# fgiral000/gencast-flax-nnx

Measured on AMD Instinct MI355X. Metric: denoiser-calls/sec, higher is better.
Workload: dtype f16x3 (every product = 3 fp16 MFMAs on hi/lo-split f32 operands: 22-bit products, f32 accumulate; f32 storage); 1 GPU; nano-GenCast DPM-Solver++2S 20-step sample, 2.5deg grid (73x144), 1 ensemble member per GPU, batch 1; dead_call_skipped=True, grid_nodes=10512, mesh_nodes=2562, latent=256, layers=16, heads=4, ffw_hidden=2048, c_in=262, c_out=82, k_hop=8, parallelism=ensemble-dp1, broadcast=none, rccl_ranks=0, precision=f16x3, library_built_from_this_tree=True, launcher=single

## Files before the change

### gencast-flax-nnx_amd/csrc/gc_api.hip

```cpp
#include <dlfcn.h>

#include "gc_handle.h"

using namespace gci;

namespace {

void protect_pending_noise(gc_handle* h) {
  if (h->guard_pending && h->d_noise == h->last_noise) std::swap(h->d_noise, h->d_noise_alt);
}

int check_ready(gc_handle* h) {
  if (!h) return GC_ERR_INVALID_ARGUMENT;
  if (!h->finalized) return fail(h, GC_ERR_STATE, "gc_finalize has not been called");
  return GC_OK;
}

struct Rccl {
  void* lib = nullptr;
  ncclResult_t (*GetUniqueId)(ncclUniqueId*) = nullptr;
  ncclResult_t (*CommInitRank)(ncclComm_t*, int, ncclUniqueId, int) = nullptr;
  ncclResult_t (*CommDestroy)(ncclComm_t) = nullptr;
  ncclResult_t (*CommCount)(const ncclComm_t, int*) = nullptr;
  ncclResult_t (*CommUserRank)(const ncclComm_t, int*) = nullptr;
// ... 104 lines not shown
  return hipDeviceGetPCIBusId(out, (int)cap, device_id) == hipSuccess ? GC_OK : GC_ERR_HIP;
}

const char* gc_last_error(const gc_handle* h) { return h ? h->err.c_str() : g_create_error.c_str(); }

static void read_switches(gc_handle* h) {
  auto is = [](const char* name, const char* value) { const char* v = std::getenv(name); return v && std::string(v) == value; };
  auto off = [](const char* name) { const char* v = std::getenv(name); return v && *v && std::atoi(v) == 0; };
  auto on = [](const char* name) { const char* v = std::getenv(name); return v && *v == '1'; };
  h->f16x3 = !is("GC_PRECISION", "f32");
  h->use_graphs = !is("GC_TUNE_GRAPH", "0");
  h->m2g_fuse_sum = !off("GC_TUNE_M2G_FUSE_SUM");
  h->embed_cache = !off("GC_TUNE_EMBED_CACHE");
  h->attn_items = !off("GC_TUNE_ATTN_ITEMS");
  h->mlp_pair = !off("GC_TUNE_MLP_PAIR");
  h->edge_terms = !off("GC_TUNE_EDGE_TERMS");
  h->a16 = !off("GC_TUNE_A16");
  h->graph_serialize = on("GC_TUNE_GRAPH_SERIALIZE");
  h->graph_verbose = on("GC_TUNE_GRAPH_VERBOSE");
  h->poison = on("GC_DEBUG_POISON");
}

int gc_create(const gc_config* cfg, int device_id, gc_handle** out) {
  return guarded(nullptr, [&]() -> int {
  if (!cfg || !out) { g_create_error = "null argument"; return GC_ERR_INVALID_ARGUMENT; }
  *out = nullptr;
  const gc_config& c = *cfg;
  auto bad = [&](const char* m) { g_create_error = m; return GC_ERR_INVALID_ARGUMENT; };
  if (c.latent_size <= 0 || c.d_model <= 0 || c.num_heads <= 0 || c.ffw_hidden <= 0 ||
      c.num_layers < 0 || c.c_in <= 0 || c.c_out <= 0 || c.batch <= 0)
    return bad("all dimensions must be positive");
// ... 1228 lines not shown
```

### gencast-flax-nnx_amd/csrc/gc_forward.hip

```cpp
#include "gc_handle.h"

namespace gci {

template <class To, class From>
static const To& a16_view(const From& v) {
  static_assert(sizeof(To) == sizeof(From), "argument struct mismatch between the two kernel builds");
  return reinterpret_cast<const To&>(v);
}

Route make_route(const gc_handle* h) {
  const int D = h->cfg.d_model, F = h->cfg.ffw_hidden;
  Route r;
  r.f16 = h->f16x3 && !h->weights_f16_unsafe && !h->in_fallback;
  r.x32 = !r.f16 && h->f32_ws;
  const bool streams = r.f16 || r.x32;
  r.ffw_slabs = streams ? h->ffw_fused_slabs : 0;
  r.st16 = h->feat16 && h->a16 && r.f16 && D % 128 == 0 && D <= 512 &&
           (h->ffw_fused_slabs > 0 || (F % 128 == 0 && (F / h->ffw2_splits) % 128 == 0));
  r.v2 = r.f16 && r.ws(3 * D, D, 1);
  r.att_items = (h->att_n_items > 0 && r.ws(3 * D, D, 1) && h->attn_splits == 1 && D <= 512) ? h->att_n_items : 0;
  r.fuse_row = streams && D % 128 == 0 && D <= 512;
  r.node_ws = r.f16;
  r.split_edge = h->split_edge;
  r.try_pair = h->mlp_pair && h->hidden_layers == 1;
  r.m2g_fused = h->m2g_fuse_sum && h->hg.m2g_tri && h->hidden_layers == 1 && streams;
  r.embed_cache = h->embed_cache_live && h->embed_cache_ready && !h->feat16 && h->hidden_layers == 1 && streams;
  r.edge_terms = h->embed_cache_live && h->terms.ready && edge_terms_possible(h) && r.f16;
  return r;
}

bool edge_terms_possible(const gc_handle* h) {
  return h->edge_terms && h->f16x3 && !h->weights_f16_unsafe && !h->in_fallback && !h->feat16 && h->hidden_layers == 1 &&
         h->cfg.latent_size == 256 && h->cfg.batch == 1 && h->hg.m2g_tri;
}

static gc::Segment seg(const float* ptr, const int* index, const float* affine, int width, int ld, int bcast) {
  gc::Segment s;
  s.ptr = ptr; s.index = index; s.affine = affine; s.width = width; s.ld = ld; s.bcast = bcast;
  return s;
}

struct MlpCall {
// ... 13 lines not shown
                        const float* residual = nullptr) {
  MlpCall c;
  c.rows = rows; c.B = B; c.out = out; c.ldo = ldo; c.residual = residual;
  return c.segments(segs);
}

static int build_mlp_args(gc_handle* h, const DevMlp& w, const MlpCall& c, gc::MlpArgs* out_args) {
  const Route& r = h->route;
  gc::MlpArgs& a = *out_args;
  a = gc::MlpArgs{};
  a.nseg = c.nseg; a.nadd = c.nadd;
  std::copy(c.seg, c.seg + c.nseg, a.seg);
  std::copy(c.add, c.add + c.nadd, a.add);
  a.rows = c.rows; a.B = c.B; a.hidden = h->cfg.latent_size;
  a.f16 = r.f16 ? 1 : 0;
  const Weight& w1 = c.nadd ? w.w1e : w.w1;
  a.w1t = pick(w1, r, Form::Staged); a.ldw1 = w1.ld; a.b1 = w.b1;
  a.w2t = pick(w.w2, r, Form::Staged); a.b2 = w.b2;
  if (r.f16 || r.x32) {
    a.w1f = pick(w1, r, Form::Streaming); a.k1f = w1.kf;
    a.w2f = pick(w.w2, r, Form::Streaming); a.ones = h->d_ones; a.zeros = h->d_zeros;
    a.f32w = r.x32 ? 1 : 0;
  }
  a.n_out = w.n_out; a.n_out_pad = w.n_out_pad; a.do_ln = c.ln ? 1 : 0;
  a.cond = (c.cond && w.cond_off >= 0) ? (h->cond_cur ? h->cond_cur : h->d_cond) + w.cond_off : nullptr;
  a.cond_stride = h->cond_total;
  a.residual = c.residual; a.out = c.out; a.ldo = c.ldo;
  a.round16 = h->feat16 ? 1 : 0;
  a.round_out = (h->feat16 && c.round_out) ? 1 : 0;
  a.a16 = r.st16 ? 1 : 0;
  a.seg0_f32 = c.seg0_f32 ? 1 : 0;
  a.out_f32 = c.out_f32 ? 1 : 0;
  a.tri = c.tri ? 1 : 0;
  if (c.tri && !gc::mlp_runs_weight_streaming(a))
    return fail(h, GC_ERR_INTERNAL, "the triple-sum epilogue exists in the weight-streaming MLP kernel only");
  return GC_OK;
}

static int enqueue_mlp(gc_handle* h, const gc::MlpArgs& a) {
  return launch(h, gc::KC_MLP, [&] {
    return a.a16 ? gc_a16::launch_mlp(h->stream, a16_view<gc_a16::MlpArgs>(a)) : gc::launch_mlp(h->stream, a);
  });
}
static int enqueue_mlp_pair(gc_handle* h, const gc::MlpArgs& a, const gc::MlpArgs& b) {
  return launch(h, gc::KC_MLP, [&] {
    return a.a16 ? gc_a16::launch_mlp_pair(h->stream, a16_view<gc_a16::MlpArgs>(a), a16_view<gc_a16::MlpArgs>(b))
                 : gc::launch_mlp_pair(h->stream, a, b);
  });
}
static int enqueue_gemm_ws(gc_handle* h, int cls, const gc::GemmArgs& ga, int mt, int splits, int epi) {
  return launch(h, cls, [&] {
    return ga.a16 ? gc_a16::launch_gemm_ws(h->stream, cls, a16_view<gc_a16::GemmArgs>(ga), mt, splits, epi)
                  : gc::launch_gemm_ws(h->stream, cls, ga, mt, splits, epi);
  });
}
static int enqueue_gemm_rowop(gc_handle* h, int cls, const gc::GemmArgs& ga, const gc::RowFuse& rf) {
  return launch(h, cls, [&] {
    return ga.a16 ? gc_a16::launch_gemm_rowop(h->stream, cls, a16_view<gc_a16::GemmArgs>(ga), a16_view<gc_a16::RowFuse>(rf))
                  : gc::launch_gemm_rowop(h->stream, cls, ga, rf);
  });
}
static int enqueue_ffw_fused(gc_handle* h, const gc::FfwArgs& fa) {
// ... 86 lines not shown
static int node_gemm(gc_handle* h, const float* nodes, int rows, const Weight& w, float* out) {
  const Route& r = h->route;
  const int L = h->cfg.latent_size;
  gc::GemmArgs ga{};
  ga.a = nodes; ga.lda = L; ga.a_f32 = 1; ga.ldw = L;
  ga.rows = rows; ga.n = L; ga.k_slice = L; ga.bias = nullptr; ga.act = 0; ga.out = out; ga.ldo = L;
  ga.round16 = 0;
  ga.out_f32 = 1;
  if (r.node_ws) {
    ga.wt = pick(w, r, Form::Streaming); ga.a16 = r.st16 ? 1 : 0;
    return enqueue_gemm_ws(h, gc::KC_GEMM_NODE, ga, pick_ws_mt(rows, L, 1), 1, 0);
  }
  ga.wt = pick(w, r, Form::Staged);
  return launch(h, gc::KC_GEMM_NODE, [&] { return gc::launch_gemm(h->stream, gc::KC_GEMM_NODE, ga, 1, 0, r.f16); });
}
static int edge_node_products(gc_handle* h, const DevMlp& w, const float* senders, int snd_rows, float* snd_out,
                              const float* receivers, int rcv_rows, float* rcv_out) {
  if (int rc = node_gemm(h, senders, snd_rows, w.w1snd, snd_out)) return rc;
  return node_gemm(h, receivers, rcv_rows, w.w1rcv, rcv_out);
}

static MlpCall edge_call(gc_handle* h, const float* e_hat, const float* e_affine, int E, const int* snd, const int* rcv,
                         const float* nsnd, const float* nrcv, const float* psnd, const float* prcv, float* out) {
  const int B = h->cfg.batch, L = h->cfg.latent_size;
  MlpCall c = mlp_call({seg(e_hat, nullptr, e_affine, L, L, 1)}, E * B, B, out, L);
  c.seg0_f32 = true;
  if (h->route.split_edge) c.add_terms({{psnd, snd}, {prcv, rcv}});
  else c.segments({seg(nsnd, snd, nullptr, L, L, 0), seg(nrcv, rcv, nullptr, L, L, 0)});
  return c;
}
// ... 65 lines not shown
                                  : mlp_call({seg(h->d_xp, nullptr, nullptr, h->kp, h->kp, 0)}, g.G * B, B, h->d_g0, L);
    embed.seg0_f32 = true;
    if (r.embed_cache) embed.add_terms({{h->d_pstat, nullptr}});
    if ((rc = run_mlp(h, r.embed_cache ? h->g2m_embed_grid_n : h->g2m_embed_grid, embed))) return rc;
  }
  const size_t ML = (size_t)g.M * L;
  if (r.edge_terms && (h->term_slot < 0 || !h->terms.ready))
    return fail(h, GC_ERR_INTERNAL, "edge terms: the forward has no slot of the cache");
  const float* const m0 = r.edge_terms ? h->terms.m0 + h->term_slot * ML : h->d_m0;
  h->m0_cur = m0;
  if (!r.edge_terms && (rc = launch(h, gc::KC_PACK, [&] {
         return gc::launch_affine_rows(s, h->d_m0_hat, cond + h->g2m_embed_mesh.cond_off, cs, g.M, B, L,
                                       h->d_m0, h->feat16, r.st16);
       })))
    return rc;
  if (r.edge_terms && (rc = node_gemm(h, h->d_g0, g.G * B, h->g2m_edge.w1snd, h->d_pg))) return rc;
  const MlpCall edge = r.edge_terms
                           ? edge_terms_call(h, h->terms.T1 + (size_t)h->term_slot * g.E1 * L, g.E1, h->d_g2m_snd, h->d_g2m_rcv,
                                             h->d_pg, h->terms.Pm + h->term_slot * ML, h->d_e1)
                           : edge_call(h, h->d_e0_hat, cond + h->g2m_embed_edge.cond_off, g.E1, h->d_g2m_snd, h->d_g2m_rcv,
                                       h->d_g0, h->d_m0, h->d_pg, h->d_pm, h->d_e1);
  const MlpCall node = mlp_call({seg(h->d_g0, nullptr, nullptr, L, L, 0)}, g.G * B, B, h->d_g1, L, h->d_g0);
  gc::MlpArgs ea{}, na{};
  bool paired = false;
  if (r.try_pair) {
    if ((rc = build_mlp_args(h, h->g2m_edge, edge, &ea)) || (rc = build_mlp_args(h, h->g2m_grid, node, &na))) return rc;
    paired = gc::mlp_pair_supported(ea, na);
  }
  if (r.split_edge && (rc = edge_node_products(h, h->g2m_edge, h->d_g0, g.G * B, h->d_pg, h->d_m0, g.M * B, h->d_pm)))
    return rc;
  if ((rc = paired ? enqueue_mlp_pair(h, ea, na) : run_mlp(h, h->g2m_edge, edge))) return rc;
  if ((rc = launch(h, gc::KC_SEGSUM, [&] {
         return gc::launch_segsum(s, h->d_e1, h->d_g2m_ptr, h->d_g2m_eid, g.M, g.E1, B, L, h->d_agg1, h->feat16, r.st16,
                                  h->g2m_agg_norm);
       })))
    return rc;
  if ((rc = run_mlp(h, h->g2m_mesh, mlp_call({seg(m0, nullptr, nullptr, L, L, 0), seg(h->d_agg1, nullptr, nullptr, L, L, 0)},
// ... 151 lines not shown
  const gc::HostGraph& g = h->hg;
  const gc_config& c = h->cfg;
  const size_t L = c.latent_size, n = distinct.size();
  const size_t per_slot = ((size_t)g.E1 + g.E2 + 2 * (size_t)g.M) * L;
  t.bytes = (int64_t)(n * per_slot * sizeof(float));
  if (n == 0 || n > (size_t)gc::kMaxSigmaList || t.bytes > h->edge_term_cap_mb * (int64_t)(1 << 20) ||
      n * (size_t)c.batch * h->cond_total > h->cond_all_cap) {
    t.bytes = 0;
    return GC_OK;
  }
  int rc;
  BufferGroup* own = &h->term_allocs;
  if ((rc = dev_alloc(h, &t.T1, n * g.E1 * L, own)) || (rc = dev_alloc(h, &t.T2, n * g.E2 * L, own)) ||
      (rc = dev_alloc(h, &t.m0, n * g.M * L, own)) || (rc = dev_alloc(h, &t.Pm, n * g.M * L, own)))
    return rc;
  hipStream_t s = h->stream;
  h->route = make_route(h);
  gc::SigmaList sl{};
  for (size_t i = 0; i < n; ++i) sl.v[i] = distinct[i];
  if ((rc = launch(h, gc::KC_COND, [&] {
         return gc::launch_cond_multi(s, sl, (int)n, c.batch, h->d_nw0t, h->d_nb0, h->d_nw1t, h->d_nb1, c.noise_num_frequencies,
                                      c.noise_hidden, c.noise_base_period, h->d_wc_all, h->d_bc_all, h->cond_total, h->d_cond_all);
       })))
    return rc;
  const int cs = h->cond_total;
  for (size_t i = 0; i < n; ++i) {
    const float* cond = h->d_cond_all + i * (size_t)c.batch * cs;
    const struct { const float* hat; int cond_off, items; float* staged; const Weight* w; float* out; } passes[] = {
        {h->d_e0_hat, h->g2m_embed_edge.cond_off, g.E1, h->d_e1, &h->g2m_edge.w1e, t.T1 + i * g.E1 * L},
        {h->d_f0_hat, h->m2g_embed_edge.cond_off, g.E2, h->d_f1, &h->m2g_edge.w1e, t.T2 + i * g.E2 * L},
// ... 15 lines not shown
```

### gencast-flax-nnx_amd/csrc/gc_handle.h

```cpp
#pragma once
#include <hip/hip_runtime.h>

#include <algorithm>
#include <array>
#include <cmath>
#include <cstdio>
#include <cstdlib>
#include <cstring>
#include <map>
#include <memory>
#include <mutex>
#include <string>
#include <type_traits>
#include <vector>

#include <rccl/rccl.h>

#include "../../include/gencast_hip.h"
#include "../../include/gencast_hip_debug.h"
#include "gc_graph.h"
#include "gc_kernels.h"

namespace gci {

// ... 1 lines not shown

struct Route {
  bool f16 = false;
  bool x32 = false;
  bool st16 = false;
  int ffw_slabs = 0;
  bool v2 = false;
  int att_items = 0;
  bool fuse_row = false;
  bool node_ws = false;
  bool m2g_fused = false;
  bool split_edge = false;
  bool try_pair = false;
  bool embed_cache = false;
  bool edge_terms = false;
  bool ws(int n, int k, int splits) const { return (f16 || x32) && n % 128 == 0 && (k / splits) % 128 == 0; }
};

struct Weight {
  float* t = nullptr;
  float* s = nullptr;
  float* f = nullptr;
  float* x = nullptr;
  int ld = 0, kf = 0;
};
enum class Form { Staged, Streaming };
inline const float* pick(const Weight& w, const Route& r, Form form) {
  if (form == Form::Streaming) return r.x32 ? w.x : w.f;
  return r.f16 ? w.s : w.t;
}
// ... 115 lines not shown
  float *d_wc_all = nullptr, *d_bc_all = nullptr;

  float *d_m0_hat = nullptr, *d_e0_hat = nullptr, *d_f0_hat = nullptr;

  int kp = 0;
  float *d_sigma = nullptr, *d_condvec = nullptr, *d_cond = nullptr;
  float* d_cond_all = nullptr;
  size_t cond_all_cap = 0;
  const float* cond_cur = nullptr;
  float *d_feats = nullptr, *d_xp = nullptr, *d_g0 = nullptr, *d_g1 = nullptr, *d_m0 = nullptr,
        *d_x = nullptr, *d_e1 = nullptr, *d_agg1 = nullptr, *d_qkv = nullptr, *d_att = nullptr,
        *d_u = nullptr, *d_m2 = nullptr, *d_f1 = nullptr, *d_agg2 = nullptr, *d_g2 = nullptr,
        *d_y = nullptr, *d_h = nullptr, *d_part = nullptr, *d_apart_o = nullptr, *d_apart_ml = nullptr,
        *d_pg = nullptr, *d_pm = nullptr;
  bool mlp_pair = true;
  bool embed_cache = true;
  bool embed_cache_ready = false;
  bool embed_cache_live = false;
  int nwp = 0;
  float *d_xn = nullptr, *d_pstat = nullptr;
  float *w1st_t = nullptr, *w1st_s = nullptr;
  gci::DevMlp g2m_embed_grid_n;
  std::vector<int> h_slots;
  int64_t embed_cache_samples = 0;
  bool m2g_fuse_sum = true;
  struct EdgeTerms {
    bool ready = false;
    std::vector<float> sigmas;
    std::vector<int> call_slot;
    float *T1 = nullptr, *T2 = nullptr, *m0 = nullptr, *Pm = nullptr;
    int64_t bytes = 0;
  };
  bool edge_terms = true;
  int64_t edge_term_cap_mb = 4096;
  EdgeTerms terms;
  gci::BufferGroup term_allocs{groups};
  int term_slot = -1;
  const float* m0_cur = nullptr;
  int64_t edge_term_samples = 0;
  float *d_ones = nullptr, *d_zeros = nullptr;
  int hidden_layers = 1;
  float* d_mlp_tmp[2] = {nullptr, nullptr};
  float *d_feats2 = nullptr, *d_ro_a = nullptr, *d_ro_b = nullptr, *d_ro_forc = nullptr;
  int *d_ro_kind = nullptr, *d_ro_src = nullptr, *d_ro_sidx = nullptr;
  int ro_nforc = -1, ro_forc_cap = 0;
  bool has_sample = false;
  int max_tile_chunks = 0;
  int ffw_fused_slabs = 0;
// ... 463 lines not shown
```

### gencast-flax-nnx_amd/csrc/gc_kernels.hip

```cpp
#include "gc_kernels.h"

#include <algorithm>
#include <atomic>
#include <type_traits>

#include <math.h>
#include <stdlib.h>

#ifdef GC_TU_A16
#define GC_TU_NS gc_a16
#else
#define GC_TU_NS gc
#endif
namespace GC_TU_NS {
#ifdef GC_TU_A16
constexpr bool kTuA16 = true;
#else
constexpr bool kTuA16 = false;
#endif

#include "gc_dev_common.inc"


struct DynLdsOnce {
// ... 1034 lines not shown
          if (c + e < n) a.out[(size_t)orow * a.ldo + c + e] = v[e];
      }
    }
  }
  });
}

template <int NT1, int NT2, int MT, int WM, int NWC = 4, int NW2 = NWC,
          int OCC = mlp_ws_occ<NT1, WM, NWC>() , bool A16 = false,
          bool F32 = false, bool TERMS = false>
__global__ __launch_bounds__(64 * NWC * WM, OCC) void gc_mlp_ws_kernel(MlpArgs a) {
  gc_mlp_ws_body<NT1, NT2, MT, WM, NWC, NW2, OCC, A16, F32, TERMS>(a, (int)blockIdx.x);
}

template <int NT1, int NT2, int MT, int WM, int NWC = 4, int NW2 = NWC,
          int OCC = mlp_ws_occ<NT1, WM, NWC>(), bool A16 = false, bool F32 = false, bool TERMS_A = false >
__global__ __launch_bounds__(64 * NWC * WM, OCC) void gc_mlp_ws_pair_kernel(MlpArgs a, MlpArgs b, int na) {
  if ((int)blockIdx.x < na) gc_mlp_ws_body<NT1, NT2, MT, WM, NWC, NW2, OCC, A16, F32, TERMS_A>(a, (int)blockIdx.x);
  else gc_mlp_ws_body<NT1, NT2, MT, WM, NWC, NW2, OCC, A16, F32>(b, (int)blockIdx.x - na);
}

template <int NT1, int NT2, int MT, int WM, int NWC, int NW2>
static hipError_t mlp_ws_geometry(const MlpArgs& a, int* grid_out, size_t* lds_out) {
  constexpr int HID = NT1 * 32 * NWC, NPAD = NT2 * 32 * NW2, BM = 32 * MT * WM;
  constexpr int abuf = 2 * BM * ((BM >= 128 ? 64 : 128) + 4);
  constexpr int region = (abuf > BM * (HID + 4)) ? abuf : BM * (HID + 4);
  static_assert(BM * (NPAD + 4) <= region, "output tile must fit the shared region");
  *lds_out = (size_t)(6 * BM + region) * sizeof(float);
  if (a.nadd < 0 || a.nadd > 3 || (a.nadd > 0 && !a.add[0].ptr) || (a.nadd > 1 && !a.add[1].ptr) || (a.nadd > 2 && !a.add[2].ptr))
    return hipErrorInvalidValue;
  if (a.nseg != 0 && a.nadd > 2) return hipErrorInvalidValue;
  int ksum = 0;
  for (int i = 0; i < a.nseg; ++i) {
    if (a.seg[i].width % 32 || a.seg[i].ld % 4) return hipErrorInvalidValue;
// ... 11 lines not shown
      if (h16 && (a.seg[i].affine || a.seg[i].ld % 8 || a.seg[i].width % 8)) return hipErrorInvalidValue;
      if (a.nseg > 1 && a.seg[i].width % KCc) return hipErrorInvalidValue;
    }
  }
  int grid = (a.rows + BM - 1) / BM;
  if (a.tri) {
    if (a.rows % 3 || a.residual || a.ldo % 4 || a.n_out % 4 ||
        (a.cond && ((reinterpret_cast<size_t>(a.cond) & 15) || a.cond_stride % 4)))
      return hipErrorInvalidValue;
    grid = (a.rows / 3 + BM / 3 - 1) / (BM / 3);
  }
  *grid_out = grid;
  return hipSuccess;
}

template <int NT1, int NT2, int MT, int WM, int NWC = 4, int NW2 = NWC, bool TERMS_A = false>
static hipError_t launch_mlp_ws_pair_t(hipStream_t s, const MlpArgs& a, const MlpArgs& b) {
  int ga = 0, gb = 0;
  size_t lds = 0;
  if (hipError_t e = mlp_ws_geometry<NT1, NT2, MT, WM, NWC, NW2>(a, &ga, &lds)) return e;
  if (hipError_t e = mlp_ws_geometry<NT1, NT2, MT, WM, NWC, NW2>(b, &gb, &lds)) return e;
  constexpr int OCC = mlp_ws_occ<NT1, WM, NWC>();
  if ((a.nseg == 0) != TERMS_A || b.nseg == 0) return hipErrorInvalidValue;
  if constexpr (TERMS_A) {
    if constexpr (kTuA16) return hipErrorInvalidValue;
    else {
      static DynLdsOnce once_t;
      if (hipError_t e = once_t.ensure((const void*)gc_mlp_ws_pair_kernel<NT1, NT2, MT, WM, NWC, NW2, OCC, false, false, true>, (int)lds)) return e;
      hipLaunchKernelGGL((gc_mlp_ws_pair_kernel<NT1, NT2, MT, WM, NWC, NW2, OCC, false, false, true>), dim3(ga + gb),
                         dim3(64 * NWC * WM), lds, s, a, b, ga);
      return hipGetLastError();
    }
  }
  if constexpr (!kTuA16) {
    if (a.f32w) {
      static DynLdsOnce once32;
      if (hipError_t e = once32.ensure((const void*)gc_mlp_ws_pair_kernel<NT1, NT2, MT, WM, NWC, NW2, OCC, false, true>, (int)lds)) return e;
      hipLaunchKernelGGL((gc_mlp_ws_pair_kernel<NT1, NT2, MT, WM, NWC, NW2, OCC, false, true>), dim3(ga + gb),
                         dim3(64 * NWC * WM), lds, s, a, b, ga);
      return hipGetLastError();
    }
  }
  static DynLdsOnce once;
  if (hipError_t e = once.ensure((const void*)gc_mlp_ws_pair_kernel<NT1, NT2, MT, WM, NWC, NW2, OCC, kTuA16>, (int)lds)) return e;
  hipLaunchKernelGGL((gc_mlp_ws_pair_kernel<NT1, NT2, MT, WM, NWC, NW2, OCC, kTuA16>), dim3(ga + gb),
                     dim3(64 * NWC * WM), lds, s, a, b, ga);
  return hipGetLastError();
}

template <int NT1, int NT2, int MT, int WM, int NWC = 4, int NW2 = NWC, bool TERMS = false>
static hipError_t launch_mlp_ws_t(hipStream_t s, const MlpArgs& a) {
  int grid = 0;
  size_t lds = 0;
  if (hipError_t e = mlp_ws_geometry<NT1, NT2, MT, WM, NWC, NW2>(a, &grid, &lds)) return e;
  constexpr int OCC = mlp_ws_occ<NT1, WM, NWC>();
  if ((a.nseg == 0) != TERMS) return hipErrorInvalidValue;
  if constexpr (TERMS) {
    if constexpr (kTuA16) return hipErrorInvalidValue;
    else {
      static DynLdsOnce once_t;
      if (hipError_t e = once_t.ensure((const void*)gc_mlp_ws_kernel<NT1, NT2, MT, WM, NWC, NW2, OCC, false, false, true>, (int)lds)) return e;
// ... 58 lines not shown
  if (a.f16 || a.a16 || a.tri || !a.w1t || a.nadd < 0 || a.nadd > 2 || a.nseg == 0) return hipErrorInvalidValue;
  for (int i = 0; i < a.nadd; ++i)
    if (!a.add[i].index) return hipErrorInvalidValue;
#define GC_MLP(A_, B_) \
  if (nt1 == A_ && nt2 == B_) return launch_mlp_t<A_, B_, false, 1>(s, a);
  GC_MLP(1, 1) GC_MLP(2, 2) GC_MLP(2, 1) GC_MLP(4, 4) GC_MLP(4, 1)
#undef GC_MLP
  return hipErrorInvalidValue;
}

bool mlp_pair_supported(const MlpArgs& a, const MlpArgs& b) {
  auto ok = [](const MlpArgs& m) {
    if (!mlp_runs_weight_streaming(m) || m.tri || m.n_out_pad != m.hidden) return false;
    return m.hidden == 512 || (m.hidden == 256 && m.rows < kMlpMt2Rows);
  };
  if (b.nseg == 0 || (a.nseg == 0 && a.hidden != 256)) return false;
  return ok(a) && ok(b) && a.hidden == b.hidden && a.f16 == b.f16 && a.f32w == b.f32w && a.a16 == b.a16;
}
hipError_t launch_mlp_pair(hipStream_t s, const MlpArgs& a, const MlpArgs& b) {
  if (!mlp_pair_supported(a, b)) return hipErrorInvalidValue;
  if (a.hidden == 512) return launch_mlp_ws_pair_t<2, 2, 2, 1, 8, 8>(s, a, b);
  if (a.nseg == 0) return launch_mlp_ws_pair_t<1, 1, 1, 1, 8, 8, true>(s, a, b);
  return launch_mlp_ws_pair_t<1, 1, 1, 1, 8, 8>(s, a, b);
}

template <bool H16>
__device__ __forceinline__ f32x4 seg_ld4(const float* base, size_t elem) {
  if constexpr (H16) return ldh4(as_h16(base) + elem);
  else return ld4(base + elem);
}
template <bool H16>
__device__ __forceinline__ void seg_st4(float* base, size_t elem, f32x4 v) {
  if constexpr (H16) sth4(as_h16(base) + elem, v);
  else st4(base + elem, v);
}

template <bool H16>
__global__ __launch_bounds__(256) void gc_segsum_kernel(const float* __restrict__ src,
// ... 753 lines not shown
        }
        if (grow < g.rows) {
          if (g.out_f32) st4(g.out + (size_t)grow * g.ldo + cb + 8 * j, v);
          else sth4(as_h16(g.out) + (size_t)grow * g.ldo + cb + 8 * j, v);
        }
      }
    }
#ifdef GC_STAMPS
    stamp_out();
#endif
    return;
  }
  float bias_v = bias_reg;
  asm volatile("" : "+v"(bias_v));
  float* obase = (EPI == 1 ? g.out + (size_t)z * g.rows * g.ldo : g.out) + ntile * BN + wave * 32 + r;
  auto emit = [&](auto full_c, auto act_c, auto rnd_c) {
    constexpr bool FULL = decltype(full_c)::value, ACT = decltype(act_c)::value, RND = decltype(rnd_c)::value;
#pragma unroll
    for (int mt = 0; mt < MT; ++mt) {
      const int row0 = mtile * BM + mt * 32;
#pragma unroll
      for (int q = 0; q < 16; ++q) {
        float v = hilo(acc[mt][q], acc2[mt][q]);
        const int grow = row0 + acc_row(q, hh);
        if (EPI != 1) {
          v += bias_v;
          if (ACT) v = gelu_tanh_fast(v);
        }
        if (!F32 && CLS == KC_GEMM_QKV && EPI == 0) v = (fabsf(v) <= kF16Max) ? v : __builtin_nanf("");
        if (EPI != 1) v = r16_c<RND>(v);
// ... 12 lines not shown
  else emit(std::false_type{}, std::false_type{}, std::false_type{});
#ifdef GC_STAMPS
  stamp_out();
#endif
}

template <int CLS>
static hipError_t launch_gemm_ws_c(hipStream_t s, const GemmArgs& g_in, int mt, int splits, int epi) {
  if ((mt != 1 && mt != 2) || epi < 0 || (epi > 1 && epi != 3)) return hipErrorInvalidValue;
  if (epi == 3 && (CLS != KC_GEMM_QKV || !g_in.kv16 || g_in.kv_d % 32 || g_in.n != 3 * g_in.kv_d || splits != 1 ||
                   g_in.att_S > 0 || g_in.bias))
    return hipErrorInvalidValue;
  const int KC = mt == 1 ? 256 : 128;
  const int kc = g_in.k_slice < KC ? g_in.k_slice : KC;
  if (g_in.n % 128 || kc % 64 || g_in.k_slice % 128 || g_in.k_slice % kc || g_in.lda % 4 || g_in.ldw % 16 || splits < 1)
    return hipErrorInvalidValue;
  GemmArgs g = g_in;
  g.splits = splits;
  const int BM = 32 * mt;
  const int total = ((g.rows + BM - 1) / BM) * (g.n / 128) * splits;
  if (total <= 0) return hipSuccess;
  dim3 grid((total + 7) / 8 * 8), block(256);
#define GC_WS(MT_, EPI_, AM_) \
  hipLaunchKernelGGL((gc_gemm_ws_kernel<MT_, EPI_, CLS, AM_, 4, 3, kTuA16, (kTuA16 && AM_ == 0 && MT_ == 2)>), grid, block, 0, s, g);
  if constexpr (!kTuA16) {
    if (g.f32w) {
#define GC_WS32(MT_, EPI_, AM_) hipLaunchKernelGGL((gc_gemm_ws_kernel<MT_, EPI_, CLS, AM_, 4, 3, false, false, true>), grid, block, 0, s, g);
      if (epi == 3) return hipErrorInvalidValue;
      if (g.att_S > 0) {
        if (mt != 1 || epi != 1 || g.att_S > kMaxAttnSplits) return hipErrorInvalidValue;
// ... 1726 lines not shown
```

### gencast-flax-nnx_amd/csrc/gc_kernels_decl.inc

```
namespace GC_KERNELS_NS {

enum KernelClass : int {
  KC_COND = 0,
  KC_PACK,
  KC_MLP,
  KC_SEGSUM,
  KC_ROWOP,
  KC_GEMM_QKV,
  KC_ATTN,
  KC_ATTN_COMBINE,
  KC_GEMM_OUT,
  KC_GEMM_FFW1,
  KC_GEMM_FFW2,
  KC_GEMM_NODE,
  KC_NOISE,
  KC_COUNT
};

constexpr int kTileM = 32;
constexpr int kCondDim = 16;

struct Segment {
  const float* ptr;
  const int* index;
// ... 48 lines not shown
hipError_t launch_cond(hipStream_t s, const float* sigma_dev, float sigma_scalar, int B,
                       const float* w0t, const float* b0, const float* w1t, const float* b1,
                       int nfreq, int nhid, float base_period,
                       const float* wc_all, const float* bc_all, int total, float* cond_vec,
                       float* cond_out);

constexpr int kMaxSigmaList = 96;
struct SigmaList { float v[kMaxSigmaList]; };
hipError_t launch_cond_multi(hipStream_t s, const SigmaList& sl, int ncalls, int B, const float* w0t,
                             const float* b0, const float* w1t, const float* b1, int nfreq, int nhid,
                             float base_period, const float* wc_all, const float* bc_all, int total,
                             float* cond_out);

hipError_t launch_mlp(hipStream_t s, const MlpArgs& a);
bool mlp_pair_supported(const MlpArgs& a, const MlpArgs& b);
hipError_t launch_mlp_pair(hipStream_t s, const MlpArgs& a, const MlpArgs& b);

hipError_t launch_segsum(hipStream_t s, const float* src, const int* rowptr, const int* eids,
                         int n_items, int n_edges, int B, int width, float* out, bool round16 = false,
                         bool h16 = false ,
                         float norm = 0.f );

struct GemmArgs {
  const float* a;
  int lda;
  int a_f32;
  const float* att_po;
  const float* att_pml;
  int att_S, att_B, att_H, att_DH;
  const int* att_tiles;
  const float* wt;
  int ldw;
  int rows, n;
  int k_slice;
  int splits;
  const float* bias;
  int act;
  float* out;
  int ldo;
  int round16;
  int a16;
  void* kv16;
  int kv_d;
  int out_f32;
  int f32w;
};
hipError_t launch_gemm(hipStream_t s, int cls, const GemmArgs& g, int splits, int epi, bool f16);
hipError_t launch_gemm_ws(hipStream_t s, int cls, const GemmArgs& g, int mt, int splits, int epi);
#ifdef GC_STAMPS
hipError_t set_gemm_ws_stamp_buffer(unsigned long long* p);
#endif

struct FfwArgs {
  const float* a;
  int rows, d, f;
  const float* w1f;
  const float* b1;
  const float* w2f;
  float* out;
  int round16;
// ... 92 lines not shown
```

### gencast-flax-nnx_amd/csrc/gc_weights.hip

```cpp
#include "gc_handle.h"

namespace gci {

const char* const P_NOISE = "denoiser.noise_level_encoder";
const char* const P_G2M = "denoiser.predictor.grid2mesh_gnn";
const char* const P_M2G = "denoiser.predictor.mesh2grid_gnn";
const char* const P_TR = "denoiser.predictor.mesh_gnn.batch_first_transformer";

void add_mlp_specs(gc_handle* h, const std::string& p, int n_in, int n_hid, int n_out, bool cond) {
  const int nh = h->hidden_layers;
  for (int i = 0; i < nh; ++i) {
    const std::string l = p + ".network.network.layers." + std::to_string(2 * i);
    h->specs[l + ".kernel"] = {i == 0 ? n_in : n_hid, n_hid};
    h->specs[l + ".bias"] = {n_hid};
  }
  const std::string l = p + ".network.network.layers." + std::to_string(2 * nh);
  h->specs[l + ".kernel"] = {n_hid, n_out};
  h->specs[l + ".bias"] = {n_out};
  if (cond) {
    h->specs[p + ".norm_conditioning_layer.conditional_linear_layer.kernel"] = {gc::kCondDim, 2 * n_out};
    h->specs[p + ".norm_conditioning_layer.conditional_linear_layer.bias"] = {2 * n_out};
  }
}

// ... 241 lines not shown
  if ((rc = dev_upload(h, &n.w1e.f, encode_wf16(wn, L, k1e), own))) return rc;
  if (h->f32_ws && (rc = dev_upload(h, &n.w1e.x, encode_wf32(wn, L, k1e), own))) return rc;
  if (!h->d_xn) {
    const size_t GB = (size_t)h->hg.G * c.batch;
    if ((rc = dev_alloc(h, &h->d_xn, GB * h->nwp))) return rc;
    if ((rc = dev_alloc(h, &h->d_pstat, GB * L))) return rc;
    GC_HIP(h, hipMemset(h->d_xn, 0, GB * h->nwp * sizeof(float)));
  }
  h->embed_cache_ready = true;
  return GC_OK;
}

void free_weights(gc_handle* h) {
  (void)drop_edge_terms(h);
  h->weight_allocs.free();
  h->finalized = h->finalized_weights = h->embed_cache_ready = false;
  h->cond_cur = nullptr;
}

int finalize_weights(gc_handle* h) {
  const gc_config& c = h->cfg;
  const int L = c.latent_size, D = c.d_model, F = c.ffw_hidden;
  const std::string g = P_G2M, m = P_M2G, t = P_TR, nz = P_NOISE;
  BufferGroup* own = &h->weight_allocs;
  CondPacker cp;
  int rc;
  const int node_in = 3 + c.c_in;
  const std::string gn = g + ".processor_networks.0.graph_network";
  const std::string gn2 = m + ".processor_networks.0.graph_network";
  if (h->hidden_layers >= 2) {
// ... 10 lines not shown
  if ((rc = upload_mlp(h, gn + ".update_edge_fns.grid2mesh.edge_fn", 3 * L, 0, 3 * L, 3 * L, L, L, true, &cp, &h->g2m_edge))) return rc;
  if ((rc = upload_mlp(h, gn + ".update_node_fns.mesh_nodes.node_fn", 2 * L, 0, 2 * L, 2 * L, L, L, true, &cp, &h->g2m_mesh))) return rc;
  if ((rc = upload_mlp(h, gn + ".update_node_fns.grid_nodes.node_fn", L, 0, L, L, L, L, true, &cp, &h->g2m_grid))) return rc;
  if ((rc = upload_mlp(h, m + ".embedder_network.embed_edge_fns.mesh2grid", 4, 0, 4, 32, L, L, true, &cp, &h->m2g_embed_edge))) return rc;
  if ((rc = upload_mlp(h, gn2 + ".update_edge_fns.mesh2grid.edge_fn", 3 * L, 0, 3 * L, 3 * L, L, L, true, &cp, &h->m2g_edge))) return rc;
  if ((rc = upload_mlp(h, gn2 + ".update_node_fns.grid_nodes.node_fn", 2 * L, 0, 2 * L, 2 * L, L, L, true, &cp, &h->m2g_grid))) return rc;
  if ((rc = upload_mlp(h, m + ".decoder_network.embed_node_fns.grid_nodes", L, 0, L, L, L, c.c_out, false, &cp, &h->m2g_dec))) return rc;

  for (DevMlp* em : {&h->g2m_edge, &h->m2g_edge}) {
    const std::string pth = (em == &h->g2m_edge) ? gn + ".update_edge_fns.grid2mesh.edge_fn"
                                                 : gn2 + ".update_edge_fns.mesh2grid.edge_fn";
    const auto& k1 = h->weights.at(pth + ".network.network.layers.0.kernel");
    if ((rc = upload_weight(h, transpose_pad(k1, 3 * L, L, 0, L, L, L), L, L, L, h->f32_ws, &em->w1e))) return rc;
    if ((rc = upload_weight(h, transpose_pad(k1, 3 * L, L, L, L, L, L), L, L, L, false, &em->w1snd))) return rc;
    if ((rc = upload_weight(h, transpose_pad(k1, 3 * L, L, 2 * L, L, L, L), L, L, L, false, &em->w1rcv))) return rc;
  }
  h->layers.assign(c.num_layers, DevLayer());
  for (int i = 0; i < c.num_layers; ++i) {
    const std::string b = t + ".blocks." + std::to_string(i);
    DevLayer& ly = h->layers[i];
    auto wt = [&](const char* name, int n_in, int n_out) {
      return transpose_pad(h->weights.at(b + name), n_in, n_out, 0, n_in, n_in, n_out);
    };
    std::vector<float> qkv((size_t)3 * D * D);
    int part = 0;
    for (const char* q : {"q", "k", "v"}) {
      const auto tt = wt((std::string(".attn_module.") + q + "_proj.linear.kernel").c_str(), D, D);
      std::copy(tt.begin(), tt.end(), qkv.begin() + (size_t)part++ * D * D);
    }
    if ((rc = upload_weight(h, qkv, 3 * D, D, D, h->f32_ws, &ly.wqkv))) return rc;
// ... 46 lines not shown
```

Before: 781.2 calls/s.

## Fuse grid-node first-layer GEMM with edge sender products and reorder MLP pair blocks

Concatenates the grid2mesh edge sender weight and the grid node MLP first-layer weight into one image. One node GEMM with a split output now produces both the sender products and a precomputed node term Pn. The grid node MLP then consumes Pn as an add-term rather than recomputing its first layer, and the pair kernel gains a form where both halves use terms. It also adds an option to launch the heavier (terms-form or larger-K) half of an MLP pair first, to improve block scheduling. The change adds a buffer of size G×L and more template instantiations, and it changes the block-index mapping in the pair kernel.

```diff
diff --git a/gencast-flax-nnx_amd/csrc/gc_api.hip b/gencast-flax-nnx_amd/csrc/gc_api.hip
--- a/gencast-flax-nnx_amd/csrc/gc_api.hip
+++ b/gencast-flax-nnx_amd/csrc/gc_api.hip
@@ -142,7 +142,9 @@
   h->embed_cache = !off("GC_TUNE_EMBED_CACHE");
   h->attn_items = !off("GC_TUNE_ATTN_ITEMS");
   h->mlp_pair = !off("GC_TUNE_MLP_PAIR");
+  h->pair_order = !off("GC_TUNE_PAIR_ORDER");
   h->edge_terms = !off("GC_TUNE_EDGE_TERMS");
+  h->node_terms = !off("GC_TUNE_NODE_TERMS");
   h->a16 = !off("GC_TUNE_A16");
   h->graph_serialize = on("GC_TUNE_GRAPH_SERIALIZE");
   h->graph_verbose = on("GC_TUNE_GRAPH_VERBOSE");
diff --git a/gencast-flax-nnx_amd/csrc/gc_forward.hip b/gencast-flax-nnx_amd/csrc/gc_forward.hip
--- a/gencast-flax-nnx_amd/csrc/gc_forward.hip
+++ b/gencast-flax-nnx_amd/csrc/gc_forward.hip
@@ -26,6 +26,7 @@
   r.m2g_fused = h->m2g_fuse_sum && h->hg.m2g_tri && h->hidden_layers == 1 && streams;
   r.embed_cache = h->embed_cache_live && h->embed_cache_ready && !h->feat16 && h->hidden_layers == 1 && streams;
   r.edge_terms = h->embed_cache_live && h->terms.ready && edge_terms_possible(h) && r.f16;
+  r.node_terms = r.edge_terms && h->node_terms && h->w1sn_f && h->terms.Pn;
   return r;
 }
 
@@ -69,7 +70,7 @@
   std::copy(c.add, c.add + c.nadd, a.add);
   a.rows = c.rows; a.B = c.B; a.hidden = h->cfg.latent_size;
   a.f16 = r.f16 ? 1 : 0;
-  const Weight& w1 = c.nadd ? w.w1e : w.w1;
+  const Weight& w1 = (c.nadd && w.w1e.kf) ? w.w1e : w.w1;
   a.w1t = pick(w1, r, Form::Staged); a.ldw1 = w1.ld; a.b1 = w.b1;
   a.w2t = pick(w.w2, r, Form::Staged); a.b2 = w.b2;
   if (r.f16 || r.x32) {
@@ -98,9 +99,10 @@
   });
 }
 static int enqueue_mlp_pair(gc_handle* h, const gc::MlpArgs& a, const gc::MlpArgs& b) {
+  const bool b_first = h->pair_order && gc::mlp_pair_second_leads(a, b);
   return launch(h, gc::KC_MLP, [&] {
-    return a.a16 ? gc_a16::launch_mlp_pair(h->stream, a16_view<gc_a16::MlpArgs>(a), a16_view<gc_a16::MlpArgs>(b))
-                 : gc::launch_mlp_pair(h->stream, a, b);
+    return a.a16 ? gc_a16::launch_mlp_pair(h->stream, a16_view<gc_a16::MlpArgs>(a), a16_view<gc_a16::MlpArgs>(b), b_first)
+                 : gc::launch_mlp_pair(h->stream, a, b, b_first);
   });
 }
 static int enqueue_gemm_ws(gc_handle* h, int cls, const gc::GemmArgs& ga, int mt, int splits, int epi) {
@@ -217,6 +219,15 @@
   ga.wt = pick(w, r, Form::Staged);
   return launch(h, gc::KC_GEMM_NODE, [&] { return gc::launch_gemm(h->stream, gc::KC_GEMM_NODE, ga, 1, 0, r.f16); });
 }
+static int node_gemm2(gc_handle* h, const float* nodes, int rows, const float* image, float* out_a, float* out_b) {
+  const int L = h->cfg.latent_size;
+  gc::GemmArgs ga{};
+  ga.a = nodes; ga.lda = L; ga.a_f32 = 1; ga.ldw = L;
+  ga.rows = rows; ga.n = 2 * L; ga.k_slice = L; ga.bias = nullptr; ga.act = 0; ga.out = out_a; ga.ldo = L;
+  ga.out2 = out_b; ga.n_out1 = L;
+  ga.round16 = 0; ga.out_f32 = 1; ga.wt = image;
+  return enqueue_gemm_ws(h, gc::KC_GEMM_NODE, ga, pick_ws_mt(rows, 2 * L, 1), 1, 0);
+}
 static int edge_node_products(gc_handle* h, const DevMlp& w, const float* senders, int snd_rows, float* snd_out,
                               const float* receivers, int rcv_rows, float* rcv_out) {
   if (int rc = node_gemm(h, senders, snd_rows, w.w1snd, snd_out)) return rc;
@@ -312,13 +323,19 @@
                                        h->d_m0, h->feat16, r.st16);
        })))
     return rc;
-  if (r.edge_terms && (rc = node_gemm(h, h->d_g0, g.G * B, h->g2m_edge.w1snd, h->d_pg))) return rc;
+  if (r.edge_terms && (rc = r.node_terms ? node_gemm2(h, h->d_g0, g.G * B, h->w1sn_f, h->d_pg, h->terms.Pn)
+                                         : node_gemm(h, h->d_g0, g.G * B, h->g2m_edge.w1snd, h->d_pg)))
+    return rc;
   const MlpCall edge = r.edge_terms
                            ? edge_terms_call(h, h->terms.T1 + (size_t)h->term_slot * g.E1 * L, g.E1, h->d_g2m_snd, h->d_g2m_rcv,
                                              h->d_pg, h->terms.Pm + h->term_slot * ML, h->d_e1)
                            : edge_call(h, h->d_e0_hat, cond + h->g2m_embed_edge.cond_off, g.E1, h->d_g2m_snd, h->d_g2m_rcv,
                                        h->d_g0, h->d_m0, h->d_pg, h->d_pm, h->d_e1);
-  const MlpCall node = mlp_call({seg(h->d_g0, nullptr, nullptr, L, L, 0)}, g.G * B, B, h->d_g1, L, h->d_g0);
+  MlpCall node = mlp_call({seg(h->d_g0, nullptr, nullptr, L, L, 0)}, g.G * B, B, h->d_g1, L, h->d_g0);
+  if (r.node_terms) {
+    node = mlp_call({}, g.G * B, B, h->d_g1, L, h->d_g0);
+    node.add_terms({{h->terms.Pn, nullptr}});
+  }
   gc::MlpArgs ea{}, na{};
   bool paired = false;
   if (r.try_pair) {
@@ -500,6 +517,7 @@
   if ((rc = dev_alloc(h, &t.T1, n * g.E1 * L, own)) || (rc = dev_alloc(h, &t.T2, n * g.E2 * L, own)) ||
       (rc = dev_alloc(h, &t.m0, n * g.M * L, own)) || (rc = dev_alloc(h, &t.Pm, n * g.M * L, own)))
     return rc;
+  if (h->node_terms && h->w1sn_f && (rc = dev_alloc(h, &t.Pn, (size_t)g.G * c.batch * L, own))) return rc;
   hipStream_t s = h->stream;
   h->route = make_route(h);
   gc::SigmaList sl{};
diff --git a/gencast-flax-nnx_amd/csrc/gc_handle.h b/gencast-flax-nnx_amd/csrc/gc_handle.h
--- a/gencast-flax-nnx_amd/csrc/gc_handle.h
+++ b/gencast-flax-nnx_amd/csrc/gc_handle.h
@@ -39,6 +39,7 @@
   bool try_pair = false;
   bool embed_cache = false;
   bool edge_terms = false;
+  bool node_terms = false;
   bool ws(int n, int k, int splits) const { return (f16 || x32) && n % 128 == 0 && (k / splits) % 128 == 0; }
 };
 
@@ -184,6 +185,7 @@
         *d_y = nullptr, *d_h = nullptr, *d_part = nullptr, *d_apart_o = nullptr, *d_apart_ml = nullptr,
         *d_pg = nullptr, *d_pm = nullptr;
   bool mlp_pair = true;
+  bool pair_order = true;
   bool embed_cache = true;
   bool embed_cache_ready = false;
   bool embed_cache_live = false;
@@ -199,9 +201,12 @@
     std::vector<float> sigmas;
     std::vector<int> call_slot;
     float *T1 = nullptr, *T2 = nullptr, *m0 = nullptr, *Pm = nullptr;
+    float* Pn = nullptr;
     int64_t bytes = 0;
   };
   bool edge_terms = true;
+  bool node_terms = true;
+  float* w1sn_f = nullptr;
   int64_t edge_term_cap_mb = 4096;
   EdgeTerms terms;
   gci::BufferGroup term_allocs{groups};
diff --git a/gencast-flax-nnx_amd/csrc/gc_kernels.hip b/gencast-flax-nnx_amd/csrc/gc_kernels.hip
--- a/gencast-flax-nnx_amd/csrc/gc_kernels.hip
+++ b/gencast-flax-nnx_amd/csrc/gc_kernels.hip
@@ -1072,10 +1072,12 @@
 }
 
 template <int NT1, int NT2, int MT, int WM, int NWC = 4, int NW2 = NWC,
-          int OCC = mlp_ws_occ<NT1, WM, NWC>(), bool A16 = false, bool F32 = false, bool TERMS_A = false >
-__global__ __launch_bounds__(64 * NWC * WM, OCC) void gc_mlp_ws_pair_kernel(MlpArgs a, MlpArgs b, int na) {
-  if ((int)blockIdx.x < na) gc_mlp_ws_body<NT1, NT2, MT, WM, NWC, NW2, OCC, A16, F32, TERMS_A>(a, (int)blockIdx.x);
-  else gc_mlp_ws_body<NT1, NT2, MT, WM, NWC, NW2, OCC, A16, F32>(b, (int)blockIdx.x - na);
+          int OCC = mlp_ws_occ<NT1, WM, NWC>(), bool A16 = false, bool F32 = false, bool TERMS_A = false ,
+          bool TERMS_B = false >
+__global__ __launch_bounds__(64 * NWC * WM, OCC) void gc_mlp_ws_pair_kernel(MlpArgs a, MlpArgs b, int na, int a0, int b0) {
+  const int ta = (int)blockIdx.x - a0;
+  if ((unsigned)ta < (unsigned)na) gc_mlp_ws_body<NT1, NT2, MT, WM, NWC, NW2, OCC, A16, F32, TERMS_A>(a, ta);
+  else gc_mlp_ws_body<NT1, NT2, MT, WM, NWC, NW2, OCC, A16, F32, TERMS_B>(b, (int)blockIdx.x - b0);
 }
 
 template <int NT1, int NT2, int MT, int WM, int NWC, int NW2>
@@ -1117,21 +1119,23 @@
   return hipSuccess;
 }
 
-template <int NT1, int NT2, int MT, int WM, int NWC = 4, int NW2 = NWC, bool TERMS_A = false>
-static hipError_t launch_mlp_ws_pair_t(hipStream_t s, const MlpArgs& a, const MlpArgs& b) {
+template <int NT1, int NT2, int MT, int WM, int NWC = 4, int NW2 = NWC, bool TERMS_A = false, bool TERMS_B = false>
+static hipError_t launch_mlp_ws_pair_t(hipStream_t s, const MlpArgs& a, const MlpArgs& b, bool b_first) {
   int ga = 0, gb = 0;
   size_t lds = 0;
   if (hipError_t e = mlp_ws_geometry<NT1, NT2, MT, WM, NWC, NW2>(a, &ga, &lds)) return e;
   if (hipError_t e = mlp_ws_geometry<NT1, NT2, MT, WM, NWC, NW2>(b, &gb, &lds)) return e;
   constexpr int OCC = mlp_ws_occ<NT1, WM, NWC>();
-  if ((a.nseg == 0) != TERMS_A || b.nseg == 0) return hipErrorInvalidValue;
+  static_assert(TERMS_A || !TERMS_B, "a second half in the terms form: only beside a first one");
+  if ((a.nseg == 0) != TERMS_A || (b.nseg == 0) != TERMS_B) return hipErrorInvalidValue;
+  const int a0 = b_first ? gb : 0, b0 = b_first ? 0 : ga;
   if constexpr (TERMS_A) {
     if constexpr (kTuA16) return hipErrorInvalidValue;
     else {
       static DynLdsOnce once_t;
-      if (hipError_t e = once_t.ensure((const void*)gc_mlp_ws_pair_kernel<NT1, NT2, MT, WM, NWC, NW2, OCC, false, false, true>, (int)lds)) return e;
-      hipLaunchKernelGGL((gc_mlp_ws_pair_kernel<NT1, NT2, MT, WM, NWC, NW2, OCC, false, false, true>), dim3(ga + gb),
-                         dim3(64 * NWC * WM), lds, s, a, b, ga);
+      if (hipError_t e = once_t.ensure((const void*)gc_mlp_ws_pair_kernel<NT1, NT2, MT, WM, NWC, NW2, OCC, false, false, true, TERMS_B>, (int)lds)) return e;
+      hipLaunchKernelGGL((gc_mlp_ws_pair_kernel<NT1, NT2, MT, WM, NWC, NW2, OCC, false, false, true, TERMS_B>), dim3(ga + gb),
+                         dim3(64 * NWC * WM), lds, s, a, b, ga, a0, b0);
       return hipGetLastError();
     }
   }
@@ -1140,14 +1144,14 @@
       static DynLdsOnce once32;
       if (hipError_t e = once32.ensure((const void*)gc_mlp_ws_pair_kernel<NT1, NT2, MT, WM, NWC, NW2, OCC, false, true>, (int)lds)) return e;
       hipLaunchKernelGGL((gc_mlp_ws_pair_kernel<NT1, NT2, MT, WM, NWC, NW2, OCC, false, true>), dim3(ga + gb),
-                         dim3(64 * NWC * WM), lds, s, a, b, ga);
+                         dim3(64 * NWC * WM), lds, s, a, b, ga, a0, b0);
       return hipGetLastError();
     }
   }
   static DynLdsOnce once;
   if (hipError_t e = once.ensure((const void*)gc_mlp_ws_pair_kernel<NT1, NT2, MT, WM, NWC, NW2, OCC, kTuA16>, (int)lds)) return e;
   hipLaunchKernelGGL((gc_mlp_ws_pair_kernel<NT1, NT2, MT, WM, NWC, NW2, OCC, kTuA16>), dim3(ga + gb),
-                     dim3(64 * NWC * WM), lds, s, a, b, ga);
+                     dim3(64 * NWC * WM), lds, s, a, b, ga, a0, b0);
   return hipGetLastError();
 }
 
@@ -1236,14 +1240,19 @@
     if (!mlp_runs_weight_streaming(m) || m.tri || m.n_out_pad != m.hidden) return false;
     return m.hidden == 512 || (m.hidden == 256 && m.rows < kMlpMt2Rows);
   };
-  if (b.nseg == 0 || (a.nseg == 0 && a.hidden != 256)) return false;
+  if ((a.nseg == 0 && a.hidden != 256) || (b.nseg == 0 && a.nseg != 0)) return false;
   return ok(a) && ok(b) && a.hidden == b.hidden && a.f16 == b.f16 && a.f32w == b.f32w && a.a16 == b.a16;
 }
-hipError_t launch_mlp_pair(hipStream_t s, const MlpArgs& a, const MlpArgs& b) {
+bool mlp_pair_second_leads(const MlpArgs& a, const MlpArgs& b) {
+  if ((a.nseg == 0) != (b.nseg == 0)) return a.nseg == 0;
+  return b.k1f > a.k1f;
+}
+hipError_t launch_mlp_pair(hipStream_t s, const MlpArgs& a, const MlpArgs& b, bool b_first) {
   if (!mlp_pair_supported(a, b)) return hipErrorInvalidValue;
-  if (a.hidden == 512) return launch_mlp_ws_pair_t<2, 2, 2, 1, 8, 8>(s, a, b);
-  if (a.nseg == 0) return launch_mlp_ws_pair_t<1, 1, 1, 1, 8, 8, true>(s, a, b);
-  return launch_mlp_ws_pair_t<1, 1, 1, 1, 8, 8>(s, a, b);
+  if (a.hidden == 512) return launch_mlp_ws_pair_t<2, 2, 2, 1, 8, 8>(s, a, b, b_first);
+  if (a.nseg == 0 && b.nseg == 0) return launch_mlp_ws_pair_t<1, 1, 1, 1, 8, 8, true, true>(s, a, b, b_first);
+  if (a.nseg == 0) return launch_mlp_ws_pair_t<1, 1, 1, 1, 8, 8, true>(s, a, b, b_first);
+  return launch_mlp_ws_pair_t<1, 1, 1, 1, 8, 8>(s, a, b, b_first);
 }
 
 template <bool H16>
@@ -2027,6 +2036,10 @@
   float bias_v = bias_reg;
   asm volatile("" : "+v"(bias_v));
   float* obase = (EPI == 1 ? g.out + (size_t)z * g.rows * g.ldo : g.out) + ntile * BN + wave * 32 + r;
+  if constexpr (EPI == 0 && CLS == KC_GEMM_NODE) {
+    if (g.out2 && ntile * BN >= g.n_out1)
+      obase = g.out2 + (ntile * BN - g.n_out1) + wave * 32 + r;
+  }
   auto emit = [&](auto full_c, auto act_c, auto rnd_c) {
     constexpr bool FULL = decltype(full_c)::value, ACT = decltype(act_c)::value, RND = decltype(rnd_c)::value;
 #pragma unroll
@@ -2069,6 +2082,8 @@
   const int KC = mt == 1 ? 256 : 128;
   const int kc = g_in.k_slice < KC ? g_in.k_slice : KC;
   if (g_in.n % 128 || kc % 64 || g_in.k_slice % 128 || g_in.k_slice % kc || g_in.lda % 4 || g_in.ldw % 16 || splits < 1)
+    return hipErrorInvalidValue;
+  if (g_in.out2 && (kTuA16 || CLS != KC_GEMM_NODE || epi != 0 || g_in.att_S > 0 || g_in.n_out1 % 128 || g_in.n_out1 <= 0 || g_in.n_out1 >= g_in.n))
     return hipErrorInvalidValue;
   GemmArgs g = g_in;
   g.splits = splits;
diff --git a/gencast-flax-nnx_amd/csrc/gc_kernels_decl.inc b/gencast-flax-nnx_amd/csrc/gc_kernels_decl.inc
--- a/gencast-flax-nnx_amd/csrc/gc_kernels_decl.inc
+++ b/gencast-flax-nnx_amd/csrc/gc_kernels_decl.inc
@@ -86,7 +86,8 @@
 
 hipError_t launch_mlp(hipStream_t s, const MlpArgs& a);
 bool mlp_pair_supported(const MlpArgs& a, const MlpArgs& b);
-hipError_t launch_mlp_pair(hipStream_t s, const MlpArgs& a, const MlpArgs& b);
+bool mlp_pair_second_leads(const MlpArgs& a, const MlpArgs& b);
+hipError_t launch_mlp_pair(hipStream_t s, const MlpArgs& a, const MlpArgs& b, bool b_first);
 
 hipError_t launch_segsum(hipStream_t s, const float* src, const int* rowptr, const int* eids,
                          int n_items, int n_edges, int B, int width, float* out, bool round16 = false,
@@ -116,6 +117,8 @@
   int kv_d;
   int out_f32;
   int f32w;
+  float* out2;
+  int n_out1;
 };
 hipError_t launch_gemm(hipStream_t s, int cls, const GemmArgs& g, int splits, int epi, bool f16);
 hipError_t launch_gemm_ws(hipStream_t s, int cls, const GemmArgs& g, int mt, int splits, int epi);
diff --git a/gencast-flax-nnx_amd/csrc/gc_weights.hip b/gencast-flax-nnx_amd/csrc/gc_weights.hip
--- a/gencast-flax-nnx_amd/csrc/gc_weights.hip
+++ b/gencast-flax-nnx_amd/csrc/gc_weights.hip
@@ -279,6 +279,7 @@
 void free_weights(gc_handle* h) {
   (void)drop_edge_terms(h);
   h->weight_allocs.free();
+  h->w1sn_f = nullptr;
   h->finalized = h->finalized_weights = h->embed_cache_ready = false;
   h->cond_cur = nullptr;
 }
@@ -319,6 +320,15 @@
     if ((rc = upload_weight(h, transpose_pad(k1, 3 * L, L, 0, L, L, L), L, L, L, h->f32_ws, &em->w1e))) return rc;
     if ((rc = upload_weight(h, transpose_pad(k1, 3 * L, L, L, L, L, L), L, L, L, false, &em->w1snd))) return rc;
     if ((rc = upload_weight(h, transpose_pad(k1, 3 * L, L, 2 * L, L, L, L), L, L, L, false, &em->w1rcv))) return rc;
+  }
+  h->w1sn_f = nullptr;
+  if (h->hidden_layers == 1 && L == 256) {
+    const auto& ke = h->weights.at(gn + ".update_edge_fns.grid2mesh.edge_fn.network.network.layers.0.kernel");
+    const auto& kn = h->weights.at(gn + ".update_node_fns.grid_nodes.node_fn.network.network.layers.0.kernel");
+    std::vector<float> both = transpose_pad(ke, 3 * L, L, L, L, L, L);
+    const std::vector<float> wn = transpose_pad(kn, L, L, 0, L, L, L);
+    both.insert(both.end(), wn.begin(), wn.end());
+    if ((rc = dev_upload(h, &h->w1sn_f, encode_wf16(both, 2 * L, L), own))) return rc;
   }
   h->layers.assign(c.num_layers, DevLayer());
   for (int i = 0; i < c.num_layers; ++i) {
```

Result: slower. 765.7 calls/s (-2.0%).
